# NVIDIA-ISAAC-ROS/isaac_ros_nvblox

Measured on NVIDIA H100. Metric: depth-frames/sec (TSDF+ESDF integrate, 640x480 @ 5 cm voxels), higher is better.
Workload: dtype f32

## Files before the change

include/nvblox_b200.h:

```cpp
#ifndef NVBLOX_B200_H_
#define NVBLOX_B200_H_

#include <stddef.h>
#include <stdint.h>

#ifdef __cplusplus
extern "C" {
#endif

#if defined(_WIN32)
#define NVB_API
#else
#define NVB_API __attribute__((visibility("default")))
#endif

typedef enum {
  NVB_OK = 0,
  NVB_ERR_INVALID_ARGUMENT = -1,
  NVB_ERR_CUDA = -2,
  NVB_ERR_CAPACITY = -3,
  NVB_ERR_INDEX_RANGE = -4,
  NVB_ERR_NO_DEVICE = -5,
  NVB_ERR_IO = -6
} NvbStatus;
// ... 418 lines not shown
NVB_API int32_t nvb_query_tsdf(NvbMapper* const* mappers, int32_t num_mappers, const float* xyz, int64_t n, float* out,
                               void* caller_stream);
NVB_API int32_t nvb_query_occupancy(NvbMapper* const* mappers, int32_t num_mappers, const float* xyz, int64_t n, float* out,
                                    void* caller_stream);

NVB_API int32_t nvb_mapper_last_esdf_stats(NvbMapper* m, int64_t out[8]);

NVB_API int32_t nvb_mapper_esdf_time_split(NvbMapper* m, int64_t out[4]);

NVB_API int32_t nvb_mapper_esdf_clear_blocks_read(NvbMapper* m, int64_t* out);

NVB_API int32_t nvb_mapper_esdf_split_stats(NvbMapper* m, int64_t out[2]);

NVB_API int32_t nvb_mapper_debug_phase_max(NvbMapper* m, int64_t* out, int32_t cap);

NVB_API int32_t nvb_mapper_enable_profiling(NvbMapper* m, int32_t enable);
NVB_API int32_t nvb_mapper_stage_times(NvbMapper* m, double* out_ms, int64_t* out_calls,
                                       int32_t reset);
NVB_API int64_t nvb_mapper_kernel_launches(const NvbMapper* m);

#ifdef __cplusplus
}
#endif
#endif
```

isaac_ros_nvblox_b200/_lib.py:

```python
import ctypes as C
import os

_HERE = os.path.dirname(os.path.abspath(__file__))
LIB_PATH = os.path.join(_HERE, "libnvblox_b200.so")

NVB_OK = 0
NVB_ERR_INDEX_RANGE, NVB_ERR_IO = -4, -6
NVB_MEM_HOST, NVB_MEM_DEVICE = 0, 1
NVB_LAYER_TSDF, NVB_LAYER_ESDF, NVB_LAYER_OCCUPANCY, NVB_LAYER_FREESPACE, NVB_LAYER_COLOR, NVB_LAYER_MESH = 0, 1, 2, 3, 4, 5
NVB_PROJECTIVE_TSDF, NVB_PROJECTIVE_OCCUPANCY, NVB_PROJECTIVE_TSDF_WITH_FREESPACE = 0, 1, 2
NVB_SPLIT_BACKGROUND, NVB_SPLIT_FOREGROUND, NVB_SPLIT_OVERLAY = 0, 1, 2

EXPORTED_SYMBOLS = [
    "nvb_last_error", "nvb_version", "nvb_device_count",
    "nvb_default_mapper_options", "nvb_default_tsdf_params", "nvb_default_esdf_params",
    "nvb_default_occupancy_params", "nvb_mapper_set_occupancy_params", "nvb_mapper_get_occupancy_params",
    "nvb_default_tsdf_decay_params", "nvb_mapper_set_tsdf_decay_params", "nvb_mapper_get_tsdf_decay_params",
    "nvb_default_occupancy_decay_params", "nvb_mapper_set_occupancy_decay_params",
    "nvb_mapper_get_occupancy_decay_params", "nvb_mapper_decay", "nvb_mapper_decay_exclude_last_view",
    "nvb_default_freespace_params", "nvb_mapper_set_freespace_params", "nvb_mapper_get_freespace_params",
    "nvb_mapper_update_freespace", "nvb_freespace_update_blocks",
    "nvb_mapper_mark_unobserved_free_inside_radius",
    "nvb_default_color_params", "nvb_mapper_set_color_params", "nvb_mapper_get_color_params",
    "nvb_mapper_integrate_color", "nvb_mapper_last_color_blocks", "nvb_sphere_tracer_render_depth",
    "nvb_default_esdf_slice_params", "nvb_mapper_set_esdf_slice_params", "nvb_mapper_get_esdf_slice_params",
    "nvb_mapper_update_esdf_slice", "nvb_esdf_integrate_slice_blocks", "nvb_esdf_slice_distance_image",
    "nvb_mapper_update_esdf_slice_planar", "nvb_esdf_integrate_slice_planar_blocks",
    "nvb_mapper_create", "nvb_mapper_destroy", "nvb_mapper_clear",
    "nvb_mapper_set_tsdf_params", "nvb_mapper_get_tsdf_params",
    "nvb_mapper_set_esdf_params", "nvb_mapper_get_esdf_params",
    "nvb_mapper_voxel_size", "nvb_mapper_block_size",
    "nvb_view_raycast", "nvb_mapper_integrate_depth", "nvb_mapper_integrate_depth_async",
    "nvb_mapper_update_esdf", "nvb_mapper_update_esdf_async", "nvb_esdf_integrate_blocks",
    "nvb_mapper_synchronize", "nvb_mapper_last_frame_block_count", "nvb_mapper_last_frame_blocks",
    "nvb_mapper_stream", "nvb_mapper_join_streams", "nvb_blocks_union",
    "nvb_layer_num_blocks", "nvb_layer_block_indices", "nvb_layer_slab_stats", "nvb_layer_get_blocks",
    "nvb_layer_set_blocks", "nvb_layer_block_device_ptr", "nvb_layer_block_bytes",
    "nvb_mapper_last_esdf_stats", "nvb_mapper_set_cache_last_viewpoint", "nvb_mapper_get_cache_last_viewpoint", "nvb_mapper_set_depth_preprocessing", "nvb_mapper_get_depth_preprocessing", "nvb_depth_dilate_invalid", "nvb_esdf_slice_aabb", "nvb_esdf_dense_grid_in_aabb", "nvb_esdf_slice_distance_image_in_aabb", "nvb_mapper_set_esdf_reserved_sms", "nvb_mapper_get_esdf_reserved_sms", "nvb_default_mesh_params", "nvb_mapper_set_mesh_params", "nvb_mapper_get_mesh_params", "nvb_mapper_update_mesh", "nvb_mesh_integrate_blocks", "nvb_mesh_update_color", "nvb_mesh_block_sizes", "nvb_mesh_get_blocks", "nvb_mesh_arena_stats", "nvb_mapper_append_frame_blocks", "nvb_blocks_union_segments", "nvb_blocks_union_status", "nvb_mapper_esdf_time_split", "nvb_mapper_esdf_clear_blocks_read", "nvb_mapper_debug_phase_max", "nvb_mapper_enable_profiling", "nvb_mapper_stage_times",
    "nvb_mapper_kernel_launches", "nvb_mapper_esdf_split_stats",
    "nvb_mapper_clear_outside_radius", "nvb_mapper_clear_tsdf_inside_shapes", "nvb_layer_clear_shapes",
    "nvb_mapper_get_cleared_blocks",
    "nvb_default_ground_plane_params", "nvb_mapper_set_ground_plane_params", "nvb_mapper_get_ground_plane_params",
    "nvb_mapper_compute_ground_plane", "nvb_mapper_ground_plane", "nvb_mapper_ground_plane_points", "nvb_ransac_fit_plane",
    "nvb_mapper_compute_dynamics", "nvb_mapper_remove_small_components", "nvb_mapper_dynamic_mask", "nvb_mapper_dynamic_overlay",
    "nvb_mapper_dynamic_points", "nvb_mapper_dynamics_device_buffers", "nvb_mapper_wait_for",
    "nvb_default_image_masker_params", "nvb_mapper_split_depth_image", "nvb_mapper_split_output",
    "nvb_mapper_split_device_buffers", "nvb_mapper_split_color_image",
    "nvb_layer_query_voxels", "nvb_layer_interpolate", "nvb_query_esdf", "nvb_query_tsdf", "nvb_query_occupancy",
    "nvb_mapper_save_map", "nvb_mapper_load_map", "nvb_layer_export_points",
    "nvb_default_sphere_tracer_params", "nvb_render_depth", "nvb_render_rgbd",
    "nvb_scene_render_depth", "nvb_scene_signed_distance", "nvb_scene_generate_layer", "nvb_scene_to_mapper",
]


# ... 247 lines not shown
    L.nvb_mapper_set_mesh_params.argtypes = [vp, C.POINTER(NvbMeshParams)]
    L.nvb_mapper_get_mesh_params.argtypes = [vp, C.POINTER(NvbMeshParams)]
    L.nvb_mapper_update_mesh.argtypes = [vp, C.c_int32]
    L.nvb_mesh_integrate_blocks.argtypes = [vp, C.POINTER(C.c_int32), C.c_int32, C.c_int32]
    L.nvb_mesh_update_color.argtypes = [vp, C.POINTER(C.c_int32), C.c_int32]
    L.nvb_mesh_block_sizes.argtypes = [vp, C.POINTER(C.c_int32), C.c_int32, C.POINTER(C.c_int32)]
    L.nvb_mesh_get_blocks.argtypes = [vp, C.POINTER(C.c_int32), C.c_int32, vp, vp, vp, vp, C.POINTER(C.c_int64)]
    L.nvb_mesh_arena_stats.argtypes = [vp, C.POINTER(C.c_int64)]
    L.nvb_mapper_append_frame_blocks.argtypes = [vp, vp, C.c_int32]
    L.nvb_blocks_union_segments.argtypes = [vp, vp, C.c_int32, C.c_int32, C.c_int32, vp, C.c_int32, vp, vp]
    L.nvb_blocks_union_status.argtypes = [vp, C.POINTER(C.c_int32)]
    L.nvb_mapper_esdf_time_split.argtypes = [vp, C.POINTER(C.c_int64)]
    L.nvb_mapper_esdf_clear_blocks_read.argtypes = [vp, C.POINTER(C.c_int64)]
    L.nvb_mapper_esdf_split_stats.argtypes = [vp, C.POINTER(C.c_int64)]
    L.nvb_mapper_debug_phase_max.argtypes = [vp, C.POINTER(C.c_int64), i32]
    L.nvb_mapper_enable_profiling.argtypes = [vp, i32]
    L.nvb_mapper_stage_times.argtypes = [vp, C.POINTER(C.c_double), C.POINTER(C.c_int64), i32]
    L.nvb_mapper_kernel_launches.argtypes = [vp]
    L.nvb_mapper_clear_outside_radius.argtypes = [vp, fp, f32, ip, i32, ip]
    L.nvb_mapper_clear_tsdf_inside_shapes.argtypes = [vp, C.POINTER(NvbBoundingShape), i32, ip, i32, ip]
    L.nvb_layer_clear_shapes.argtypes = [vp, i32, C.POINTER(NvbBoundingShape), i32, ip, i32, ip]
    L.nvb_mapper_get_cleared_blocks.argtypes = [vp, ip, i32, ip, i32, ip]
    L.nvb_default_ground_plane_params.argtypes = [C.POINTER(NvbGroundPlaneParams)]
    L.nvb_default_ground_plane_params.restype = None
    L.nvb_mapper_set_ground_plane_params.argtypes = [vp, C.POINTER(NvbGroundPlaneParams)]
    L.nvb_mapper_get_ground_plane_params.argtypes = [vp, C.POINTER(NvbGroundPlaneParams)]
    L.nvb_mapper_compute_ground_plane.argtypes = [vp, fp, ip]
    L.nvb_mapper_ground_plane.argtypes = [vp, fp, ip]
    L.nvb_mapper_ground_plane_points.argtypes = [vp, i32, fp, i32, ip, ip]
    L.nvb_ransac_fit_plane.argtypes = [vp, vp, i32, i32, i32, f32, fp, ip]
# ... 41 lines not shown
```

isaac_ros_nvblox_b200/csrc/nvb_api.cu:

```cuda
#include <algorithm>
#include <array>
#include <cfloat>
#include <cmath>
#include <cstdio>
#include <cstring>
#include <functional>
#include <set>
#include <string>
#include <vector>

#include "nvb_esdf_block.cuh"

using namespace nvb;

namespace {

thread_local std::string g_last_error;

int fail(int code, const std::string& msg) {
  g_last_error = msg;
  return code;
}

#define NVB_CUDA(expr)                                                                               \
// ... 312 lines not shown
  int grow(NvbMapper* m, int capacity);
  int setReservedSms(NvbMapper* m, int n);
  int reset(NvbMapper* m);
  int blocksWritten(NvbMapper* m);
  void forgetParentBoxes() { prune_ok_ = false; }
  void buildParentBoxes(const DevLayer& esdf, int n, cudaStream_t st) { launchEsdfParentBoxes(esdf, n, psum_.get(), st); }
  int reserveSliceColumns(NvbMapper* m, size_t columns);
  int reserveDeadCleared(NvbMapper* m);
  void beginUpdate() { update_seq_++; }
  EsdfCtx ctx(DeviceCounters* ctr) const;
  cudaError_t readStats(long long out[kNumEsdfStats]) const {
    return cudaMemcpy(out, stats_.get(), kNumEsdfStats * sizeof(long long), cudaMemcpyDeviceToHost);
  }
  cudaError_t readPhaseMax(int64_t* out, int n) const {
    return cudaMemcpy(out, phase_max_.get(), (size_t)n * sizeof(long long), cudaMemcpyDeviceToHost);
  }
  int driver() const { return driver_; }
  int reservedSms() const { return reserved_sms_; }

 private:
  static constexpr int kUnlinked = 0xFE;
  template <typename F>
  cudaError_t eachSlotArray(F f);
  int allocRecords(NvbMapper* m, int capacity);

  int driver_ = 1;
  int reserved_sms_ = 2;
  int split_min_k_ = 0;
  int ges_switch_ = 160;
  bool prune_default_ = false;
// ... 7 lines not shown
  DeviceArray<int> nbr_, nbr27_;
  DeviceArray<int> cand_stamp_, cand_a_, cand_b_;
  DeviceArray<unsigned char> shadow_;
  DeviceArray<unsigned char> xslab_;
  DeviceArray<int> xrec_;
  int xseg_ = 0;
  int xseg_grid_ = 0;
  DeviceArray<int> xcounts_;
  DeviceArray<unsigned long long> colset_;
  DeviceArray<int> cols_;
  DeviceArray<int> dead_cleared_xyz_;
  DeviceArray<unsigned int> clr_bits_;
  DeviceArray<long long> stats_;
  DeviceArray<unsigned int> barrier_;
  DeviceArray<unsigned long long> phase_max_;
};

class ViewCompaction {
 public:
  int create(NvbMapper* m);
  int reserve(NvbMapper* m, const ViewGrid& g);
  unsigned int* bits() const { return bits_.get(); }
  void compact(const ViewGrid& g, int4* list, int* count, bool allocate, const DevLayer& layer, const TrackerLists& tracker,
               int* error, bool clear, cudaStream_t st);

 private:
  DeviceArray<unsigned int> bits_;
  DeviceArray<unsigned long long> tile_state_;
  DeviceArray<unsigned int> ticket_;
  unsigned int ticket_base_ = 0;
// ... 495 lines not shown
  return e;
}

int EsdfState::create(NvbMapper* m, int capacity, int driver) {
  driver_ = driver;
  split_min_k_ = esdfWaveXSplitMinK();
  if (const char* e = getenv("NVB_GES_SWITCH")) ges_switch_ = atoi(e);
  const char* e = getenv("NVB_CLEAR_PRUNE");
  prune_default_ = prune_ok_ = driver == 3 && !(e && atoi(e) == 0);
  if (int rc = grow(m, capacity)) return rc;
  const int one = 1;
  NVB_CUDA(cudaMemcpyAsync(&m->counters.get()->ring_id, &one, sizeof(int), cudaMemcpyHostToDevice, m->stream));
  NVB_CUDA(clr_bits_.grow(m, 2048, 2048));
  NVB_CUDA(stats_.grow(m, kNumEsdfStats, kNumEsdfStats, 0));
  NVB_CUDA(phase_max_.grow(m, kPhaseMaxEntries, kPhaseMaxEntries, 0));
  NVB_CUDA(barrier_.grow(m, 16, 16, 0));
  return NVB_OK;
}

int EsdfState::grow(NvbMapper* m, int capacity) {
  const size_t n = capacity;
  const auto grow_slots = [&](auto& a, size_t per_slot, int fill, bool keep, bool) {
    return a.grow(m, per_slot * n, per_slot * n, fill, keep);
  };
  NVB_CUDA(eachSlotArray(grow_slots));
  if (driver_ == 2) NVB_CUDA(shadow_.grow(m, n * kEsdfBlockBytes, n * kEsdfBlockBytes));
  if (driver_ == 3) {
    NVB_CUDA(xslab_.grow(m, esdfWaveXSlabBytes(capacity), esdfWaveXSlabBytes(capacity)));
    if (int rc = allocRecords(m, capacity)) return rc;
    const size_t flags = esdfWaveXFlagBytes() / sizeof(int);
// ... 68 lines not shown
  c.clr_bits = clr_bits_.get();
  c.psum = psum_.get(), c.prune = (prune_ok_ && driver_ == 3) ? 1 : 0;
  c.nbr27 = nbr27_.get(), c.shadow = shadow_.get(), c.cand_stamp = cand_stamp_.get();
  c.xslab = xslab_.get(), c.xrec = xrec_.get(), c.xtail = ctr->xtail, c.xseg = xseg_, c.xcounts = xcounts_.get();
  c.xsplit_min_k = split_min_k_;
  c.ges_counts = ctr->ges_counts;
  c.cand_a = cand_a_.get(), c.cand_b = cand_b_.get(), c.ges_switch = ges_switch_;
  c.colset_keys = colset_.get(), c.colset_mask = colset_.size() ? (unsigned int)(colset_.size() - 1) : 0u;
  c.cols = cols_.get(), c.cols_count = &ctr->cols_count;
  c.dead_cleared_xyz = dead_cleared_xyz_.get();
  c.dead_cleared_count = dead_cleared_xyz_.get() ? &ctr->dead_cleared_count : nullptr;
  c.cleared_seq = &ctr->cleared_seq;
  c.update_seq = update_seq_;
  c.barrier = barrier_.get();
  c.phase_max = phase_max_.get();
  c.stats = stats_.get();
  return c;
}

constexpr int kHostListCap = 1 << 15;


int growTracker(NvbMapper* m, int cap) {
  const bool has[kNumBlocksToUpdateTypes] = {true, m->freespace.exists(), m->mesh.exists()};
  DeviceCounters* ctr = m->counters.get();
  int* const count[kNumBlocksToUpdateTypes] = {&ctr->todo_count, &ctr->todo_fs_count, &ctr->todo_mesh_count};
  const size_t n = cap;
  for (int k = 0; k < kNumBlocksToUpdateTypes; k++) {
    if (!has[k]) continue;
    TrackedBlocks& t = m->tracker[k];
// ... 2507 lines not shown
  NVB_CUDA(syncAll(m));
  long long s[kNumEsdfStats];
  NVB_CUDA(m->esdf_state.readStats(s));
  out[0] = s[kStatSplitCandidates], out[1] = s[kStatRestFetches];
  return NVB_OK;
}

int32_t nvb_mapper_debug_phase_max(NvbMapper* m, int64_t* out, int32_t cap) {
  if (!m || !out) return fail(NVB_ERR_INVALID_ARGUMENT, "null argument");
  NVB_CUDA(cudaSetDevice(m->device));
  NVB_CUDA(syncAll(m));
  NVB_CUDA(m->esdf_state.readPhaseMax(out, std::min(cap, (int32_t)kPhaseMaxEntries)));
  return NVB_OK;
}

int32_t nvb_mapper_enable_profiling(NvbMapper* m, int32_t enable) {
  if (!m) return fail(NVB_ERR_INVALID_ARGUMENT, "null mapper");
  NVB_CUDA(cudaSetDevice(m->device));
  NVB_CUDA(syncAll(m));
  collectStages(m);
  m->profiling = enable != 0;
  return NVB_OK;
}

int32_t nvb_mapper_stage_times(NvbMapper* m, double* out_ms, int64_t* out_calls, int32_t reset) {
  if (!m) return fail(NVB_ERR_INVALID_ARGUMENT, "null mapper");
  NVB_CUDA(cudaSetDevice(m->device));
  NVB_CUDA(syncAll(m));
  collectStages(m);
  for (int i = 0; i < kNumStages; i++) {
// ... 661 lines not shown
```

isaac_ros_nvblox_b200/csrc/nvb_esdf_wavex.cu:

```cuda
#include "nvb_esdf_wave_common.cuh"

#include <cstdlib>

namespace nvb {

namespace {

#ifndef NVB_WAVEX_THREADS
#define NVB_WAVEX_THREADS 512
#endif
#ifndef NVB_WAVEX_MAXREG
#define NVB_WAVEX_MAXREG 96
#endif
#ifndef NVB_WAVEX_TAIL
#define NVB_WAVEX_TAIL 1
#endif
#ifndef NVB_WAVEX_PROF
#define NVB_WAVEX_PROF 0
#endif
#if NVB_WAVEX_PROF
#define X_PROF_BEGIN() long long tq = clock64();
#define X_PROF(i) \
  if (lane64 == 0) xs.prof[group][i] += clock64() - tq; \
  tq = clock64();
// ... 1 lines not shown
  if (lane64 == 0) xs.prof[group][i]++;
#define X_PROF_BIN(i, j, K)                                                  \
  if (lane64 == 0) {                                                         \
    const int kb = (K) <= 256 ? 0 : ((K) <= 1040 ? 1 : 2);                   \
    const long long dt = clock64() - tq;                                     \
    xs.prof[group][i] += dt, xs.prof[group][(j) + kb] += dt, xs.prof[group][(j) + 3 + kb]++; \
  }                                                                          \
  tq = clock64();
#define X_PROF_KBIN(i, j, K)                                \
  if (lane64 == 0) {                                        \
    const int kb = (K) <= 256 ? 0 : ((K) <= 1040 ? 1 : 2);  \
    const long long dt = clock64() - tq;                    \
    xs.prof[group][i] += dt, xs.prof[group][(j) + kb] += dt; \
  }                                                         \
  tq = clock64();
#else
#define X_PROF_BEGIN()
#define X_PROF(i)
#define X_PROF_COUNT(i)
#define X_PROF_BIN(i, j, K)
#define X_PROF_KBIN(i, j, K)
#endif
constexpr int kXT = NVB_WAVEX_THREADS;
constexpr int kXG = kXT / 64;
constexpr int kRecInts = 32;
constexpr int kMaxCtas = 192;
constexpr int kRX = 110, kRY = 11;
constexpr int kRegionVox = 1100;
constexpr int kFlagBase = 4 * kRegionVox;
constexpr int kXRegionWords = (kEsdfCellWords + 1) * kRegionVox;
constexpr size_t kXSmemBytes = (size_t)kXG * kXRegionWords * sizeof(unsigned int);
constexpr int kXFaceCells = 6 * 64;
constexpr int kXFlagOff = kXFaceCells * 16;
constexpr int kXSlotBytes = kXFaceCells * (16 + 4);
#if NVB_WAVEX_PROF
constexpr int kXProfWords = 24;
constexpr int kXProfBase = kPhaseMaxEntries - kXProfWords;
#endif

struct XTables {
  unsigned int halo[8][64];
  unsigned int pair[6][4][64];
};

struct XShared {
  int rec[kXG][kRecInts];
  int nb[kXG][8];
  int pos[kXG][8];
  unsigned int mask[kXG];
  int changed[kXG];
  unsigned int live[kXG][8];
  int seg[kXG][2];
  int pre[kMaxCtas + 1];
  int warp_tot[2][8];
  int ncand, nchanged;
  int next;
  int cur[kXG];
  int seeds[kXG];
  int bcast[4];
  unsigned int generation;
  int n_bar;
  int ring;
  int swept, faces, rings, n_tail;
  int n_split, n_rest;
#if NVB_WAVEX_PROF
  long long prof[kXG][kXProfWords];
#endif
};

struct XCtx {
  unsigned char* blocks;
  int* block_index;
  DevHash hash;
  int* nbr;
  int* nbr27;
  int* cand_stamp;
  unsigned int* psum;
  int* stamp[2];
  unsigned char* X[2];
  int* recs[2];
  int seg;
  int split_min_k;
  int* error;
  float max_sq;
  __device__ __forceinline__ int* segment(int p, int cta) const { return recs[p] + (size_t)cta * seg * kRecInts; }
};

__shared__ XTables x_tab;
__shared__ XShared x_xs;
__shared__ XCtx x_ctx;
extern __shared__ __align__(16) unsigned int x_smem[];

__device__ __forceinline__ int rvox(int rx, int ry, int rz) { return rx * kRX + ry * kRY + rz; }
__device__ __forceinline__ int faceEntry(int f) {
  return f == 0 ? 22 : (f == 1 ? 4 : (f == 2 ? 16 : (f == 3 ? 10 : (f == 4 ? 14 : 12))));
}
__device__ __forceinline__ int boundaryOff(int r) { return r == 0 ? -1 : (r == 9 ? 1 : 0); }
__device__ __forceinline__ int boundaryLoc(int r) { return r == 0 ? 7 : (r == 9 ? 0 : r - 1); }

// ... 386 lines not shown
  if (lane64 < 6 && s.pos >= 0) __stcg(segment + (size_t)s.pos * kRecInts, xs.nb[group][lane64]);
}

__device__ __noinline__ void processCandidate(int ring, int K) {
  const XCtx& c = x_ctx;
  const XTables& tab = x_tab;
  XShared& xs = x_xs;
  const int cta = blockIdx.x, group = threadIdx.x >> 6, lane64 = threadIdx.x & 63;
  unsigned int* R = x_smem + group * kXRegionWords;
  const int ci = ring & 1, ni = ci ^ 1;
  const bool split = K >= c.split_min_k;
  X_PROF_BEGIN()
  if (lane64 < 28) xs.rec[group][lane64] = __ldcg(c.segment(ci, xs.seg[group][0]) + (size_t)xs.seg[group][1] * kRecInts + lane64);
  groupSync(group);
  X_PROF(0)
  const int slot = xs.rec[group][0];
  const int* row = &xs.rec[group][1];
  const unsigned char* blk = c.blocks + (size_t)slot * kEsdfBlockBytes;
  int sv = ring - 1;
  if (lane64 < 27 && row[lane64] >= 0) sv = __ldcg(c.stamp[ci] + row[lane64]);
  if (split) {
    const unsigned int m = __ballot_sync(0xffffffffu, lane64 < 27 && sv == ring);
    if (lane64 == 0) xs.mask[group] = m, xs.changed[group] = 0;
  } else {
    OwnRegs own = ownLoad(blk, lane64);
    const unsigned int m = __ballot_sync(0xffffffffu, lane64 < 27 && sv == ring);
    if (lane64 == 0) xs.mask[group] = m, xs.changed[group] = 0;
    ownToShared(R, own, lane64);
  }
  groupSync(group);
// ... 25 lines not shown
      if (lane64 == 0) atomicAdd(&xs.n_rest, 1);
      cpAsyncWaitAll();
      groupSync(group);
    }
    X_PROF(8)
    sweepBlockX(R, group, lane64, c.max_sq);
    registerClaim(c, xs, rs, group, lane64, ring + 1);
    groupSync(group);
    X_PROF(4)
    ownStore(c.blocks + (size_t)slot * kEsdfBlockBytes, true, c.X[ni] + (size_t)slot * kXSlotBytes, R, c.psum + 2 * (size_t)slot, lane64);
    registerFinish(c, xs, rs, group, lane64, c.segment(ni, cta));
    X_PROF_COUNT(7)
  }
  groupSync(group);
  X_PROF_KBIN(5, 18, K)
}

__device__ __noinline__ void processSeed(int ring, int slot) {
  const XCtx& c = x_ctx;
  XShared& xs = x_xs;
  const int cta = blockIdx.x, group = threadIdx.x >> 6, lane64 = threadIdx.x & 63;
  unsigned int* R = x_smem + group * kXRegionWords;
  const int ci = ring & 1;
  unsigned char* blk = c.blocks + (size_t)slot * kEsdfBlockBytes;
  OwnRegs own = ownLoad(blk, lane64);
  if (lane64 < 6) xs.nb[group][lane64] = neighbor6(c, slot, lane64);
  if (lane64 == 0) {
    __stcg(c.stamp[ci] + slot, ring);
    xs.changed[group] = 0;
  }
  groupSync(group);
  RegState rs = registerBegin(c, xs, group, lane64, ring);
  ownToShared(R, own, lane64);
  groupSync(group);
  const bool ch = sweepBlockX(R, group, lane64, c.max_sq);
  registerClaim(c, xs, rs, group, lane64, ring);
  if (ch) xs.changed[group] = 1;
  groupSync(group);
  ownStore(blk, xs.changed[group] != 0, c.X[ci] + (size_t)slot * kXSlotBytes, R, xs.changed[group] ? c.psum + 2 * (size_t)slot : nullptr, lane64);
  registerFinish(c, xs, rs, group, lane64, c.segment(ci, cta));
  groupSync(group);
}

__device__ __forceinline__ void gridBarrierRA(unsigned int* bar, unsigned int& generation, unsigned int nctas) {
  __syncthreads();
  if (threadIdx.x == 0) {
    generation++;
    const unsigned int target = generation * nctas;
    asm volatile("red.release.gpu.global.add.u32 [%0], 1;" ::"l"(bar) : "memory");
    unsigned int v;
    do {
      asm volatile("ld.acquire.gpu.global.u32 %0, [%1];" : "=r"(v) : "l"(bar) : "memory");
    } while (v < target);
  }
  __syncthreads();
}

__device__ __forceinline__ void counterBarrierScan(XShared& xs, unsigned int* bar, unsigned int& generation, int2* counts, int nctas,
                                                   int cta, int tid, int seg, int ring_inc, int* K, int* M) {
  counts += (xs.n_bar & 1) * kMaxCtas;
  __syncthreads();
  if (tid == 0) {
    __stcg(counts + cta, make_int2(min(xs.ncand, seg), xs.nchanged));
    xs.ncand = 0, xs.nchanged = 0;
  }
  gridBarrierRA(bar, generation, nctas);
  int2 v = make_int2(0, 0);
  if (tid < nctas) v = __ldcg(counts + tid);
  const int lane = tid & 31, warp = tid >> 5;
  int inc = v.x, chg = v.y;
#pragma unroll
  for (int o = 1; o < 32; o <<= 1) {
    const int t = __shfl_up_sync(0xffffffffu, inc, o);
    if (lane >= o) inc += t;
  }
#pragma unroll
  for (int o = 16; o > 0; o >>= 1) chg += __shfl_xor_sync(0xffffffffu, chg, o);
  if (warp < 8 && lane == 31) xs.warp_tot[0][warp] = inc;
  if (warp < 8 && lane == 0) xs.warp_tot[1][warp] = chg;
  __syncthreads();
  int base = 0, mtot = 0;
#pragma unroll
  for (int w = 0; w < 8; w++) {
    if (w < warp) base += xs.warp_tot[0][w];
    if (w * 32 < nctas) mtot += xs.warp_tot[1][w];
  }
  if (tid < nctas) xs.pre[tid + 1] = base + inc;
  if (tid == 0) xs.pre[0] = 0, xs.next = 0, xs.ring += ring_inc, xs.n_bar++;
  __syncthreads();
  *K = xs.pre[nctas];
  *M = mtot;
}

__global__ void __maxnreg__(NVB_WAVEX_MAXREG) esdfWaveXKernel(EsdfCtx c) {
  XShared& xs = x_xs;
  const int cta = blockIdx.x, nctas = gridDim.x;
  const int tid = threadIdx.x, group = tid >> 6, lane64 = tid & 63;
  if (*(volatile int*)c.work_count == 0) return;
  initTables(x_tab, tid);
  if (tid == 0) {
    xs.ncand = 0, xs.nchanged = 0, xs.next = 0;
    xs.ring = *(volatile int*)c.ring_id;
    xs.generation = 0, xs.n_bar = 0, xs.swept = 0, xs.faces = 0, xs.rings = 0, xs.n_tail = 0, xs.n_split = 0, xs.n_rest = 0;
    XCtx& xc = x_ctx;
    xc.blocks = c.esdf.blocks, xc.block_index = c.esdf.block_index, xc.hash = c.esdf.hash;
    xc.nbr = c.nbr, xc.nbr27 = c.nbr27, xc.cand_stamp = c.cand_stamp, xc.psum = c.psum;
    xc.stamp[0] = c.stamp_a, xc.stamp[1] = c.stamp_b;
    xc.X[0] = c.xslab, xc.X[1] = c.xslab + (size_t)c.esdf.capacity * kXSlotBytes;
    xc.recs[0] = c.xrec, xc.recs[1] = c.xrec + (size_t)nctas * c.xseg * kRecInts;
    xc.seg = c.xseg, xc.split_min_k = c.xsplit_min_k, xc.error = c.error, xc.max_sq = c.max_sq;
  }
#if NVB_WAVEX_PROF
  if (lane64 < kXProfWords) xs.prof[group][lane64] = 0;
#endif
  __syncthreads();
#if NVB_WAVEX_PROF
  long long t_bar = 0, t_work = 0, t0 = globalTimerNs(), t1;
  int dbgK = 0, dbgM = 0;
#define X_DBG(k, m) dbgK = (k), dbgM = (m);
#define X_TIME_WORK()                                                                                                      \
  t1 = globalTimerNs(), t_work += t1 - t0;                                                                                 \
  if (tid == 0 && xs.n_bar < 1000) atomicMax((unsigned long long*)c.phase_max + xs.n_bar, (unsigned long long)(t1 - t0)); \
  if (cta == 0 && tid == 0 && xs.n_bar < 1000)                                                                             \
    c.phase_max[1000 + xs.n_bar] = dbgK, c.phase_max[2000 + xs.n_bar] = dbgM, c.phase_max[3000 + xs.n_bar] = t1 - t0;      \
  t0 = t1;
#define X_TIME_BARRIER() t1 = globalTimerNs(), t_bar += t1 - t0, t0 = t1;
#else
#define X_DBG(k, m)
#define X_TIME_WORK()
#define X_TIME_BARRIER()
#endif
#define X_BARRIER(inc, Kout, Mout)                                                                                        \
  X_TIME_WORK()                                                                                                           \
  counterBarrierScan(xs, c.barrier, xs.generation, reinterpret_cast<int2*>(c.xcounts), nctas, cta, tid, c.xseg, inc,        \
                     &(Kout), &(Mout));                                                                                   \
  X_TIME_BARRIER()
  for (int pass = 0; pass < 2; pass++) {
    const int* src = pass ? c.cleared_list : c.upd_list;
    const int n0 = pass ? *(volatile int*)c.cleared_count : *(volatile int*)c.upd_count;
    if (n0 == 0) continue;
    X_DBG(-1, n0)
    if (lane64 == 0) xs.seeds[group] = n0;
    for (;;) {
      if (lane64 == 0) xs.cur[group] = atomicAdd(&xs.next, 1);
      groupSync(group);
      const long long e = (long long)cta + (long long)xs.cur[group] * nctas;
      if (e >= xs.seeds[group]) break;
      processSeed(xs.ring, __ldcg(src + e));
    }
    int M = xs.seeds[group], K, unused;
// ... 78 lines not shown
    c.stats[kStatSlowestCtaWorkNs] = sum_max;
    for (int q = 0; q < kXProfWords; q++) c.phase_max[kXProfBase + q] = xs.prof[0][q];
#endif
  }
}

}

int esdfWaveXGrid(int num_sms, int reserved_sms) {
  int grid = num_sms < kMaxCtas ? num_sms : kMaxCtas;
  if (reserved_sms > 0 && grid - reserved_sms >= 8) grid -= reserved_sms;
  return grid;
}
size_t esdfWaveXFlagBytes() { return 2 * (size_t)kMaxCtas * sizeof(int2); }
size_t esdfWaveXSlabBytes(int capacity) { return 2 * (size_t)capacity * kXSlotBytes; }

constexpr int kSplitMinK = 0;
int esdfWaveXSplitMinK() {
  const char* e = getenv("NVB_WAVEX_SPLIT_MIN_K");
  const int v = e ? atoi(e) : kSplitMinK;
  return v < 0 ? 0 : v;
}

cudaError_t launchEsdfComputeX(const EsdfCtx& c, int num_sms, int reserved_sms, cudaStream_t stream, int* launches) {
  static int per_sm = -1;
  if (per_sm < 0) {
    cudaFuncSetAttribute(esdfWaveXKernel, cudaFuncAttributeMaxDynamicSharedMemorySize, (int)kXSmemBytes);
    int v = 0;
    if (cudaOccupancyMaxActiveBlocksPerMultiprocessor(&v, esdfWaveXKernel, kXT, kXSmemBytes) != cudaSuccess) v = 0;
    per_sm = v;
// ... 11 lines not shown
```

isaac_ros_nvblox_b200/csrc/nvb_internal.cuh:

```cuda
#pragma once
#include <cstdint>
#include <memory>
#include <string>
#include <vector>

#include <cuda_runtime.h>
#include <stdint.h>

#include "nvblox_b200.h"

namespace nvb {

constexpr int kVps = 8;
constexpr int kVpb = kVps * kVps * kVps;
constexpr int kTsdfBlockBytes = kVpb * 8;
constexpr int kEsdfBlockBytes = kVpb * (16 + 4);
constexpr int kColorBlockBytes = kVpb * 8;
constexpr int kOccBlockBytes = kVpb * 4;
constexpr int kHelperCtas = 132;

struct Vec3 {
  float x, y, z;
};

// ... 342 lines not shown
  int* cand_b;
  int ges_switch;
  int* cand_stamp;
  int* ges_counts;
  unsigned int* psum;
  unsigned int* clr_bits;
  int prune;
  int* seed_upd;
  int* seed_clr;
  int* cleared_seq;
  int update_seq;
  int* tracker_dirty;
  int* tracker_todo_count;
  unsigned int* barrier;
  unsigned long long* phase_max;
  long long* stats;
  int* error;
  float max_sq;
  float max_esdf_distance_m;
  float max_site_distance_m;
  float min_weight;
  float block_size;
  int from_occupancy;
  float occupied_threshold_log_odds;
};
void launchEsdfSliceAllocateAndMark(const EsdfCtx& c, const int* in_xyz, const int* in_slots, const int* in_count_dev,
                                    int in_count_upper, int num_sms, cudaStream_t stream);
void launchEsdfAllocate(const EsdfCtx& c, const int* in_xyz, const int* in_slots, const int* in_count_dev,
                        int in_count_upper, cudaStream_t stream);
void launchEsdfMark(const EsdfCtx& c, int count_upper, int num_sms, cudaStream_t stream);
void launchEsdfClear(const EsdfCtx& c, int esdf_count_upper, int num_sms, cudaStream_t stream);
cudaError_t launchEsdfComputeGes(const EsdfCtx& c, int num_sms, cudaStream_t stream, int* launches);
cudaError_t launchEsdfComputePersistent(const EsdfCtx& c, int num_sms, cudaStream_t stream, int* launches);
cudaError_t launchEsdfComputeX(const EsdfCtx& c, int num_sms, int reserved_sms, cudaStream_t stream, int* launches);
int esdfWaveXGrid(int num_sms, int reserved_sms);
size_t esdfWaveXFlagBytes();
size_t esdfWaveXSlabBytes(int capacity);
int esdfWaveXSplitMinK();
cudaError_t runEsdfComputeHostLoop(const EsdfCtx& c, int num_sms, cudaStream_t stream, int* launches);
int esdfPersistentMaxCtas(int num_sms);

__host__ __device__ __forceinline__ unsigned int parentBoxWord(int lo0, int hi0, int lo1, int hi1, int lo2, int hi2) {
  if (lo0 > hi0) return 0u;
  const bool fits = lo0 >= -16 && lo1 >= -16 && lo2 >= -16 && hi0 <= 15 && hi1 <= 15 && hi2 <= 15;
  return fits ? ((1u << 31) | (unsigned)(lo0 + 16) | ((unsigned)(hi0 + 16) << 5) | ((unsigned)(lo1 + 16) << 10) |
                 ((unsigned)(hi1 + 16) << 15) | ((unsigned)(lo2 + 16) << 20) | ((unsigned)(hi2 + 16) << 25))
              : 0xffffffffu;
}

constexpr int kFreespaceVoxelBytes = 24;
constexpr int kFreespaceBlockBytes = 512 * kFreespaceVoxelBytes;
#ifdef __CUDACC__
// ... 351 lines not shown
```

isaac_ros_nvblox_b200/mapper.py:

```python
import ctypes as C
import os

import numpy as np

from . import _lib
from . import io as _io
from ._lib import (NvbBoundingShape, NvbCamera, NvbDecayExclusion, NvbEsdfParams, NvbEsdfSliceParams, NvbFreespaceParams, NvbGroundPlaneParams, NvbMapperOptions, NvbOccupancyDecayParams,
                   NvbOccupancyParams, NvbTsdfDecayParams, NvbTsdfParams, check)

TSDF_VOXEL_DTYPE = np.dtype([("distance", "<f4"), ("weight", "<f4")])
ESDF_VOXEL_DTYPE = np.dtype(
    [("squared_distance_vox", "<f4"), ("parent_direction", "<i4", (3,)),
     ("is_inside", "u1"), ("observed", "u1"), ("is_site", "u1"), ("pad", "u1")])

OCCUPANCY_VOXEL_DTYPE = np.dtype([("log_odds", "<f4")])
COLOR_VOXEL_DTYPE = np.dtype([("color", "u1", (3,)), ("pad", "u1"), ("weight", "<f4")])
FREESPACE_VOXEL_DTYPE = np.dtype([("last_occupied_timestamp_ms", "<i8"), ("consecutive_occupancy_duration_ms", "<i8"),
                                  ("is_high_confidence_freespace", "u1"), ("pad", "u1", (7,))])


class ProjectiveLayerType:
    kTsdf = _lib.NVB_PROJECTIVE_TSDF
    kOccupancy = _lib.NVB_PROJECTIVE_OCCUPANCY
    kTsdfWithFreespace = _lib.NVB_PROJECTIVE_TSDF_WITH_FREESPACE
# ... 817 lines not shown
    check(mapper._L.nvb_mapper_remove_small_components(mapper._h, mask_in_ptr, mask_out_ptr, _lib.NVB_MEM_DEVICE, int(rows),
                                                        int(cols), int(threshold)))


class Mapper:

    def esdf_time_split(self):
        out = (C.c_int64 * 4)()
        check(self._L.nvb_mapper_esdf_time_split(self._h, out))
        return {"barrier_wait_ns_cta0": out[0], "axis_ns_cta0": out[1], "slowest_cta_work_ns": out[2], "barriers": out[3]}

    def debug_phase_max(self, n=4000):
        out = (C.c_int64 * n)()
        check(self._L.nvb_mapper_debug_phase_max(self._h, out, n))
        return np.frombuffer(out, dtype=np.int64).copy()

    def __init__(self, voxel_size_m, device=0, tsdf_capacity_blocks=0, esdf_capacity_blocks=0,
                 esdf_persistent=3, projective_layer_type=ProjectiveLayerType.kTsdf, keep_last_view=False):
        self._L = _lib.load()
        o = NvbMapperOptions()
        self._L.nvb_default_mapper_options(C.byref(o))
        o.voxel_size_m = float(voxel_size_m)
        o.device = int(device)
        self._device = int(device)
        if tsdf_capacity_blocks:
            o.tsdf_capacity_blocks = int(tsdf_capacity_blocks)
        if esdf_capacity_blocks:
            o.esdf_capacity_blocks = int(esdf_capacity_blocks)
        o.esdf_persistent = 1 if esdf_persistent is True else int(esdf_persistent)
        o.projective_layer_type = int(projective_layer_type)
# ... 347 lines not shown
```

Baseline: 3418.

## Fold barrier-count scan into a single warp and add handover timing probes

```diff
diff --git a/include/nvblox_b200.h b/include/nvblox_b200.h
--- a/include/nvblox_b200.h
+++ b/include/nvblox_b200.h
@@ -456,6 +456,8 @@
 
 NVB_API int32_t nvb_mapper_debug_phase_max(NvbMapper* m, int64_t* out, int32_t cap);
 
+NVB_API int32_t nvb_mapper_debug_handover(NvbMapper* m, int64_t* out, int32_t cap, int32_t* words);
+
 NVB_API int32_t nvb_mapper_enable_profiling(NvbMapper* m, int32_t enable);
 NVB_API int32_t nvb_mapper_stage_times(NvbMapper* m, double* out_ms, int64_t* out_calls,
                                        int32_t reset);
diff --git a/isaac_ros_nvblox_b200/_lib.py b/isaac_ros_nvblox_b200/_lib.py
--- a/isaac_ros_nvblox_b200/_lib.py
+++ b/isaac_ros_nvblox_b200/_lib.py
@@ -37,7 +37,7 @@
     "nvb_layer_num_blocks", "nvb_layer_block_indices", "nvb_layer_slab_stats", "nvb_layer_get_blocks",
     "nvb_layer_set_blocks", "nvb_layer_block_device_ptr", "nvb_layer_block_bytes",
     "nvb_mapper_last_esdf_stats", "nvb_mapper_set_cache_last_viewpoint", "nvb_mapper_get_cache_last_viewpoint", "nvb_mapper_set_depth_preprocessing", "nvb_mapper_get_depth_preprocessing", "nvb_depth_dilate_invalid", "nvb_esdf_slice_aabb", "nvb_esdf_dense_grid_in_aabb", "nvb_esdf_slice_distance_image_in_aabb", "nvb_mapper_set_esdf_reserved_sms", "nvb_mapper_get_esdf_reserved_sms", "nvb_default_mesh_params", "nvb_mapper_set_mesh_params", "nvb_mapper_get_mesh_params", "nvb_mapper_update_mesh", "nvb_mesh_integrate_blocks", "nvb_mesh_update_color", "nvb_mesh_block_sizes", "nvb_mesh_get_blocks", "nvb_mesh_arena_stats", "nvb_mapper_append_frame_blocks", "nvb_blocks_union_segments", "nvb_blocks_union_status", "nvb_mapper_esdf_time_split", "nvb_mapper_esdf_clear_blocks_read", "nvb_mapper_debug_phase_max", "nvb_mapper_enable_profiling", "nvb_mapper_stage_times",
-    "nvb_mapper_kernel_launches", "nvb_mapper_esdf_split_stats",
+    "nvb_mapper_kernel_launches", "nvb_mapper_esdf_split_stats", "nvb_mapper_debug_handover",
     "nvb_mapper_clear_outside_radius", "nvb_mapper_clear_tsdf_inside_shapes", "nvb_layer_clear_shapes",
     "nvb_mapper_get_cleared_blocks",
     "nvb_default_ground_plane_params", "nvb_mapper_set_ground_plane_params", "nvb_mapper_get_ground_plane_params",
@@ -315,6 +315,7 @@
     L.nvb_mapper_esdf_clear_blocks_read.argtypes = [vp, C.POINTER(C.c_int64)]
     L.nvb_mapper_esdf_split_stats.argtypes = [vp, C.POINTER(C.c_int64)]
     L.nvb_mapper_debug_phase_max.argtypes = [vp, C.POINTER(C.c_int64), i32]
+    L.nvb_mapper_debug_handover.argtypes = [vp, C.POINTER(C.c_int64), i32, C.POINTER(C.c_int32)]
     L.nvb_mapper_enable_profiling.argtypes = [vp, i32]
     L.nvb_mapper_stage_times.argtypes = [vp, C.POINTER(C.c_double), C.POINTER(C.c_int64), i32]
     L.nvb_mapper_kernel_launches.argtypes = [vp]
diff --git a/isaac_ros_nvblox_b200/csrc/nvb_api.cu b/isaac_ros_nvblox_b200/csrc/nvb_api.cu
--- a/isaac_ros_nvblox_b200/csrc/nvb_api.cu
+++ b/isaac_ros_nvblox_b200/csrc/nvb_api.cu
@@ -350,6 +350,10 @@
   }
   cudaError_t readPhaseMax(int64_t* out, int n) const {
     return cudaMemcpy(out, phase_max_.get(), (size_t)n * sizeof(long long), cudaMemcpyDeviceToHost);
+  }
+  size_t handoverWords() const { return handover_.size(); }
+  cudaError_t readHandover(int64_t* out, size_t n) const {
+    return n ? cudaMemcpy(out, handover_.get(), n * sizeof(long long), cudaMemcpyDeviceToHost) : cudaSuccess;
   }
   int driver() const { return driver_; }
   int reservedSms() const { return reserved_sms_; }
@@ -387,6 +391,7 @@
   DeviceArray<long long> stats_;
   DeviceArray<unsigned int> barrier_;
   DeviceArray<unsigned long long> phase_max_;
+  DeviceArray<long long> handover_;
 };
 
 class ViewCompaction {
@@ -912,6 +917,7 @@
   NVB_CUDA(clr_bits_.grow(m, 2048, 2048));
   NVB_CUDA(stats_.grow(m, kNumEsdfStats, kNumEsdfStats, 0));
   NVB_CUDA(phase_max_.grow(m, kPhaseMaxEntries, kPhaseMaxEntries, 0));
+  NVB_CUDA(handover_.grow(m, esdfWaveXHandoverWords(), esdfWaveXHandoverWords(), 0));
   NVB_CUDA(barrier_.grow(m, 16, 16, 0));
   return NVB_OK;
 }
@@ -1010,6 +1016,7 @@
   c.update_seq = update_seq_;
   c.barrier = barrier_.get();
   c.phase_max = phase_max_.get();
+  c.handover = handover_.get();
   c.stats = stats_.get();
   return c;
 }
@@ -3547,6 +3554,16 @@
   return NVB_OK;
 }
 
+int32_t nvb_mapper_debug_handover(NvbMapper* m, int64_t* out, int32_t cap, int32_t* words) {
+  if (!m || !out || !words) return fail(NVB_ERR_INVALID_ARGUMENT, "null argument");
+  NVB_CUDA(cudaSetDevice(m->device));
+  NVB_CUDA(syncAll(m));
+  const size_t n = std::min((size_t)std::max(cap, 0), m->esdf_state.handoverWords());
+  NVB_CUDA(m->esdf_state.readHandover(out, n));
+  *words = (int32_t)n;
+  return NVB_OK;
+}
+
 int32_t nvb_mapper_enable_profiling(NvbMapper* m, int32_t enable) {
   if (!m) return fail(NVB_ERR_INVALID_ARGUMENT, "null mapper");
   NVB_CUDA(cudaSetDevice(m->device));
diff --git a/isaac_ros_nvblox_b200/csrc/nvb_esdf_wavex.cu b/isaac_ros_nvblox_b200/csrc/nvb_esdf_wavex.cu
--- a/isaac_ros_nvblox_b200/csrc/nvb_esdf_wavex.cu
+++ b/isaac_ros_nvblox_b200/csrc/nvb_esdf_wavex.cu
@@ -39,7 +39,21 @@
     xs.prof[group][i] += dt, xs.prof[group][(j) + kb] += dt; \
   }                                                         \
   tq = clock64();
+#define X_HOV_END()                                                                     \
+  if (lane64 == 0) {                                                                    \
+    xs.gend[group][0] = globalTimerNs(), xs.gend[group][1] = clock64();                 \
+    atomicAdd(&xs.hov_n, 1);                                                            \
+  }
+#define X_HOV_REC()                                                                     \
+  if (lane64 == 0) {                                                                    \
+    atomicMin(&xs.hov[kHovRec], (long long)globalTimerNs());                            \
+    atomicMin(&xs.hov[kHovStamps + kHovRec], (long long)clock64());                     \
+  }
+#define X_HOV_STAMP(i) xs.hov[i] = globalTimerNs(), xs.hov[kHovStamps + (i)] = clock64();
 #else
+#define X_HOV_END()
+#define X_HOV_REC()
+#define X_HOV_STAMP(i)
 #define X_PROF_BEGIN()
 #define X_PROF(i)
 #define X_PROF_COUNT(i)
@@ -61,6 +75,19 @@
 #if NVB_WAVEX_PROF
 constexpr int kXProfWords = 24;
 constexpr int kXProfBase = kPhaseMaxEntries - kXProfWords;
+constexpr int kXHovPhases = 64;
+enum HovStamp {
+  kHovFirst,
+  kHovLastWork,
+  kHovLast,
+  kHovArrive,
+  kHovReleased,
+  kHovSeen,
+  kHovDealt,
+  kHovRec,
+  kHovStamps
+};
+constexpr int kXHovWords = 2 * kHovStamps + 2;
 #endif
 
 struct XTables {
@@ -77,7 +104,7 @@
   unsigned int live[kXG][8];
   int seg[kXG][2];
   int pre[kMaxCtas + 1];
-  int warp_tot[2][8];
+  int mtot;
   int ncand, nchanged;
   int next;
   int cur[kXG];
@@ -90,6 +117,9 @@
   int n_split, n_rest;
 #if NVB_WAVEX_PROF
   long long prof[kXG][kXProfWords];
+  long long hov[2 * kHovStamps];
+  long long gend[kXG][2];
+  int hov_n;
 #endif
 };
 
@@ -108,6 +138,9 @@
   int split_min_k;
   int* error;
   float max_sq;
+#if NVB_WAVEX_PROF
+  long long* handover;
+#endif
   __device__ __forceinline__ int* segment(int p, int cta) const { return recs[p] + (size_t)cta * seg * kRecInts; }
 };
 
@@ -524,6 +557,7 @@
   if (lane64 < 28) xs.rec[group][lane64] = __ldcg(c.segment(ci, xs.seg[group][0]) + (size_t)xs.seg[group][1] * kRecInts + lane64);
   groupSync(group);
   X_PROF(0)
+  X_HOV_REC()
   const int slot = xs.rec[group][0];
   const int* row = &xs.rec[group][1];
   const unsigned char* blk = c.blocks + (size_t)slot * kEsdfBlockBytes;
@@ -579,6 +613,7 @@
   }
   groupSync(group);
   X_PROF_KBIN(5, 18, K)
+  X_HOV_END()
 }
 
 __device__ __noinline__ void processSeed(int ring, int slot) {
@@ -605,56 +640,102 @@
   ownStore(blk, xs.changed[group] != 0, c.X[ci] + (size_t)slot * kXSlotBytes, R, xs.changed[group] ? c.psum + 2 * (size_t)slot : nullptr, lane64);
   registerFinish(c, xs, rs, group, lane64, c.segment(ci, cta));
   groupSync(group);
-}
-
-__device__ __forceinline__ void gridBarrierRA(unsigned int* bar, unsigned int& generation, unsigned int nctas) {
+  X_HOV_END()
+}
+
+#if NVB_WAVEX_PROF
+constexpr long long kHovNone = 0x7fffffffffffffffll;
+__device__ __forceinline__ void hovCollect(XShared& xs, int q, int cta) {
+  long long f[2] = {kHovNone, kHovNone}, l[2] = {0, 0};
+  for (int g = 0; g < kXG; g++) {
+    if (xs.gend[g][0] == 0) continue;
+    for (int k = 0; k < 2; k++) f[k] = min(f[k], xs.gend[g][k]), l[k] = max(l[k], xs.gend[g][k]), xs.gend[g][k] = 0;
+  }
+  for (int k = 0; k < 2; k++) {
+    xs.hov[k * kHovStamps + kHovFirst] = f[0] == kHovNone ? xs.hov[k * kHovStamps + kHovLast] : f[k];
+    xs.hov[k * kHovStamps + kHovLastWork] = f[0] == kHovNone ? xs.hov[k * kHovStamps + kHovLast] : l[k];
+  }
+  if (q >= 1 && q - 1 < kXHovPhases) {
+    long long* e = x_ctx.handover + ((size_t)(q - 1) * kMaxCtas + cta) * kXHovWords;
+    for (int k = 0; k < 2; k++) e[k * kHovStamps + kHovRec] = xs.hov[k * kHovStamps + kHovRec] == kHovNone ? 0 : xs.hov[k * kHovStamps + kHovRec];
+  }
+  xs.hov[kHovRec] = xs.hov[kHovStamps + kHovRec] = kHovNone;
+  if (q < kXHovPhases) {
+    long long* e = x_ctx.handover + ((size_t)q * kMaxCtas + cta) * kXHovWords;
+    e[2 * kHovStamps] = xs.hov_n, e[2 * kHovStamps + 1] = xs.nchanged;
+  }
+  xs.hov_n = 0;
+}
+__device__ __forceinline__ void hovStore(const XShared& xs, int q, int cta) {
+  if (q >= kXHovPhases) return;
+  long long* e = x_ctx.handover + ((size_t)q * kMaxCtas + cta) * kXHovWords;
+  for (int i = 0; i < 2 * kHovStamps; i++) e[i] = i % kHovStamps == kHovRec ? 0 : xs.hov[i];
+}
+#endif
+
+constexpr int kXSlotsPerLane = kMaxCtas / 32;
+static_assert(kMaxCtas % 64 == 0, "an even number of count slots per lane: 16-byte loads of two slots");
+__device__ __forceinline__ void counterBarrierScan(XShared& xs, unsigned int* bar, int2* counts, int nctas, int cta, int tid,
+                                                   int seg, int ring_inc, int* K, int* M) {
+#if NVB_WAVEX_PROF
+  const int q = xs.n_bar;
+#endif
   __syncthreads();
-  if (threadIdx.x == 0) {
-    generation++;
-    const unsigned int target = generation * nctas;
-    asm volatile("red.release.gpu.global.add.u32 [%0], 1;" ::"l"(bar) : "memory");
-    unsigned int v;
-    do {
-      asm volatile("ld.acquire.gpu.global.u32 %0, [%1];" : "=r"(v) : "l"(bar) : "memory");
-    } while (v < target);
+  if (tid < 32) {
+    counts += (xs.n_bar & 1) * kMaxCtas;
+    __syncwarp();
+    if (tid == 0) {
+#if NVB_WAVEX_PROF
+      X_HOV_STAMP(kHovLast)
+      hovCollect(xs, q, cta);
+#endif
+      __stcg(counts + cta, make_int2(min(xs.ncand, seg), xs.nchanged));
+      xs.ncand = 0, xs.nchanged = 0;
+      const unsigned int target = ++xs.generation * (unsigned int)nctas;
+      X_HOV_STAMP(kHovArrive)
+      asm volatile("red.release.gpu.global.add.u32 [%0], 1;" ::"l"(bar) : "memory");
+      X_HOV_STAMP(kHovReleased)
+      unsigned int v;
+      do {
+        asm volatile("ld.acquire.gpu.global.u32 %0, [%1];" : "=r"(v) : "l"(bar) : "memory");
+      } while (v < target);
+      X_HOV_STAMP(kHovSeen)
+    }
+    __syncwarp();
+    const int s0 = tid * kXSlotsPerLane;
+    int own = 0, chg = 0;
+    if (s0 < nctas) {
+      const int4* p = reinterpret_cast<const int4*>(counts + s0);
+#pragma unroll
+      for (int h = 0; h < kXSlotsPerLane / 2; h++) {
+        const int4 w = __ldcg(p + h);
+        if (s0 + 2 * h < nctas) xs.pre[s0 + 2 * h + 1] = w.x, own += w.x, chg += w.y;
+        if (s0 + 2 * h + 1 < nctas) xs.pre[s0 + 2 * h + 2] = w.z, own += w.z, chg += w.w;
+      }
+    }
+    int inc = own;
+#pragma unroll
+    for (int o = 1; o < 32; o <<= 1) {
+      const int t = __shfl_up_sync(0xffffffffu, inc, o);
+      if (tid >= o) inc += t;
+    }
+#pragma unroll
+    for (int o = 16; o > 0; o >>= 1) chg += __shfl_xor_sync(0xffffffffu, chg, o);
+    int run = inc - own;
+#pragma unroll
+    for (int k = 0; k < kXSlotsPerLane; k++)
+      if (s0 + k < nctas) run += xs.pre[s0 + k + 1], xs.pre[s0 + k + 1] = run;
+    if (tid == 0) xs.pre[0] = 0, xs.mtot = chg, xs.next = 0, xs.ring += ring_inc, xs.n_bar++;
   }
   __syncthreads();
-}
-
-__device__ __forceinline__ void counterBarrierScan(XShared& xs, unsigned int* bar, unsigned int& generation, int2* counts, int nctas,
-                                                   int cta, int tid, int seg, int ring_inc, int* K, int* M) {
-  counts += (xs.n_bar & 1) * kMaxCtas;
-  __syncthreads();
+#if NVB_WAVEX_PROF
   if (tid == 0) {
-    __stcg(counts + cta, make_int2(min(xs.ncand, seg), xs.nchanged));
-    xs.ncand = 0, xs.nchanged = 0;
-  }
-  gridBarrierRA(bar, generation, nctas);
-  int2 v = make_int2(0, 0);
-  if (tid < nctas) v = __ldcg(counts + tid);
-  const int lane = tid & 31, warp = tid >> 5;
-  int inc = v.x, chg = v.y;
-#pragma unroll
-  for (int o = 1; o < 32; o <<= 1) {
-    const int t = __shfl_up_sync(0xffffffffu, inc, o);
-    if (lane >= o) inc += t;
-  }
-#pragma unroll
-  for (int o = 16; o > 0; o >>= 1) chg += __shfl_xor_sync(0xffffffffu, chg, o);
-  if (warp < 8 && lane == 31) xs.warp_tot[0][warp] = inc;
-  if (warp < 8 && lane == 0) xs.warp_tot[1][warp] = chg;
-  __syncthreads();
-  int base = 0, mtot = 0;
-#pragma unroll
-  for (int w = 0; w < 8; w++) {
-    if (w < warp) base += xs.warp_tot[0][w];
-    if (w * 32 < nctas) mtot += xs.warp_tot[1][w];
-  }
-  if (tid < nctas) xs.pre[tid + 1] = base + inc;
-  if (tid == 0) xs.pre[0] = 0, xs.next = 0, xs.ring += ring_inc, xs.n_bar++;
-  __syncthreads();
+    X_HOV_STAMP(kHovDealt)
+    hovStore(xs, q, cta);
+  }
+#endif
   *K = xs.pre[nctas];
-  *M = mtot;
+  *M = xs.mtot;
 }
 
 __global__ void __maxnreg__(NVB_WAVEX_MAXREG) esdfWaveXKernel(EsdfCtx c) {
@@ -674,9 +755,15 @@
     xc.X[0] = c.xslab, xc.X[1] = c.xslab + (size_t)c.esdf.capacity * kXSlotBytes;
     xc.recs[0] = c.xrec, xc.recs[1] = c.xrec + (size_t)nctas * c.xseg * kRecInts;
     xc.seg = c.xseg, xc.split_min_k = c.xsplit_min_k, xc.error = c.error, xc.max_sq = c.max_sq;
+#if NVB_WAVEX_PROF
+    xc.handover = c.handover;
+#endif
   }
 #if NVB_WAVEX_PROF
   if (lane64 < kXProfWords) xs.prof[group][lane64] = 0;
+  if (lane64 < 2) xs.gend[group][lane64] = 0;
+  if (tid < 2 * kHovStamps) xs.hov[tid] = tid % kHovStamps == kHovRec ? kHovNone : 0;
+  if (tid == 0) xs.hov_n = 0;
 #endif
   __syncthreads();
 #if NVB_WAVEX_PROF
@@ -697,8 +784,7 @@
 #endif
 #define X_BARRIER(inc, Kout, Mout)                                                                                        \
   X_TIME_WORK()                                                                                                           \
-  counterBarrierScan(xs, c.barrier, xs.generation, reinterpret_cast<int2*>(c.xcounts), nctas, cta, tid, c.xseg, inc,        \
-                     &(Kout), &(Mout));                                                                                   \
+  counterBarrierScan(xs, c.barrier, reinterpret_cast<int2*>(c.xcounts), nctas, cta, tid, c.xseg, inc, &(Kout), &(Mout));     \
   X_TIME_BARRIER()
   for (int pass = 0; pass < 2; pass++) {
     const int* src = pass ? c.cleared_list : c.upd_list;
@@ -807,6 +893,11 @@
 }
 size_t esdfWaveXFlagBytes() { return 2 * (size_t)kMaxCtas * sizeof(int2); }
 size_t esdfWaveXSlabBytes(int capacity) { return 2 * (size_t)capacity * kXSlotBytes; }
+#if NVB_WAVEX_PROF
+size_t esdfWaveXHandoverWords() { return (size_t)kXHovPhases * kMaxCtas * kXHovWords; }
+#else
+size_t esdfWaveXHandoverWords() { return 0; }
+#endif
 
 constexpr int kSplitMinK = 0;
 int esdfWaveXSplitMinK() {
diff --git a/isaac_ros_nvblox_b200/csrc/nvb_internal.cuh b/isaac_ros_nvblox_b200/csrc/nvb_internal.cuh
--- a/isaac_ros_nvblox_b200/csrc/nvb_internal.cuh
+++ b/isaac_ros_nvblox_b200/csrc/nvb_internal.cuh
@@ -380,6 +380,7 @@
   int* tracker_todo_count;
   unsigned int* barrier;
   unsigned long long* phase_max;
+  long long* handover;
   long long* stats;
   int* error;
   float max_sq;
@@ -402,6 +403,7 @@
 int esdfWaveXGrid(int num_sms, int reserved_sms);
 size_t esdfWaveXFlagBytes();
 size_t esdfWaveXSlabBytes(int capacity);
+size_t esdfWaveXHandoverWords();
 int esdfWaveXSplitMinK();
 cudaError_t runEsdfComputeHostLoop(const EsdfCtx& c, int num_sms, cudaStream_t stream, int* launches);
 int esdfPersistentMaxCtas(int num_sms);
diff --git a/isaac_ros_nvblox_b200/mapper.py b/isaac_ros_nvblox_b200/mapper.py
--- a/isaac_ros_nvblox_b200/mapper.py
+++ b/isaac_ros_nvblox_b200/mapper.py
@@ -855,6 +855,12 @@
         out = (C.c_int64 * n)()
         check(self._L.nvb_mapper_debug_phase_max(self._h, out, n))
         return np.frombuffer(out, dtype=np.int64).copy()
+
+    def debug_handover(self, n):
+        out = (C.c_int64 * n)()
+        words = C.c_int32(0)
+        check(self._L.nvb_mapper_debug_handover(self._h, out, n, C.byref(words)))
+        return np.frombuffer(out, dtype=np.int64)[:words.value].copy()
 
     def __init__(self, voxel_size_m, device=0, tsdf_capacity_blocks=0, esdf_capacity_blocks=0,
                  esdf_persistent=3, projective_layer_type=ProjectiveLayerType.kTsdf, keep_last_view=False):
```

Result: no change. 3414 (median of 6 runs) (-0.1%).
